# TencentYoutuResearch/ImageMatching-OETR

Measured on AMD Instinct MI355X. Metric: image-pairs/sec @640x640 (OETR hot path: feature correlation + overlap regression, features resident in HBM), higher is better.
Workload: dtype f32 (3xf16-split operands, fp32 accumulate); 1 GPU; BASELINE configs[1]: batch=8 pairs/GPU, 640x640 -> 20x20 tokens/image, C=256, 8 enc + 2 dec layers, f32_split_f16; pairs_per_gpu=8, global_pairs=8, streams=3, world_size=1, gpu_max_hw_queues=4, encoder_tile_rows=64, tail_mode=direct form (throughput setting for overlapped streams), parallelism=pairs sharded over 1 rank(s); all-gather of boxes only

## Files before the change

### imagematching_oetr_amd/csrc/api.hip

```cpp
#include <math.h>
#include <stdlib.h>
#include <string.h>

#include <string>
#include <vector>

#include "../../include/oetr_hip.h"
#include "common.h"

using namespace oetr;

constexpr int OETR_PREREDUCE_MIN_TOKENS = 768;
constexpr int OETR_DIRECT_TAIL_MIN_ROWS = 16000;

namespace {

thread_local std::string g_err;

oetr_status fail(oetr_status st, const std::string& msg) {
  g_err = msg;
  return st;
}
oetr_status hip_fail(hipError_t e, const char* what) {
  return fail(OETR_ERR_HIP, std::string(what) + ": " + hipGetErrorString(e));
// ... 94 lines not shown
struct oetr_trace {
  std::vector<hipEvent_t> ev;
  std::vector<int> kid;
  int used = 0;
  int dropped = 0;
};

struct oetr_ctx {
  oetr_trace* trace = nullptr;
  int device = 0;
  int mode = GM_SPLIT;
  int kv_prereduce = -1;
  mutable int dec_fault = 0;
  int dec_split = 0;
  int tail_mode = 0;
  int policy = 0;
  int enc_tile = 0;
  int attn_full = 0;
  int num_cus = 256;
  float* dev = nullptr;
  size_t dev_floats = 0;
  EncLayerDev enc[OETR_N_ENC];
  DecKVDev dkv;
  DecLayerDev dec[OETR_N_DEC];
  const float* qe[2];
  const float *dec_tgt1, *dec_q0, *dec_qkv1;
  HeadsDev heads;
};

struct oetr_neck_ctx {
  oetr_trace* trace = nullptr;
  int device = 0;
  int num_cus = 256;
  int conv_rows = 0;
  float* dev = nullptr;
  const f32x4 *proj_wh[2], *proj_wl[2];
  const float *proj_b, *ln_w, *ln_b;
  const f32x4 *conv_wh[3], *conv_wl[3];
  const f32x4 *conv_wh_rw[3], *conv_wl_rw[3];
  int conv_kernel = 0;
  const float* conv_b[3];
  const f32x4 *out_wh, *out_wl;
  const float* out_b;
};

namespace {

#ifdef OETR_PHASE_TIMING
long long* g_tbuf = nullptr;
#endif

struct Workspace {
  float *x, *qp, *pos, *kvp[2], *ksp[2], *att0, *z0, *dkv1, *dks1, *conv_out, *gn_part, *sm_part, *hs,
      *logits, *cxy, *tlbr, *convp, *kbuf[2], *vt[2], *kvr, *ksr;
  uint32_t* flags;
  size_t bytes;
};

bool make_geom(int n, int hf1, int wf1, int hf2, int wf2, Geom* g) {
  if (n <= 0 || hf1 <= 0 || wf1 <= 0 || hf2 <= 0 || wf2 <= 0) return false;
  const long L1 = (long)hf1 * wf1, L2 = (long)hf2 * wf2;
  if (L1 > OETR_MAX_TOKENS || L2 > OETR_MAX_TOKENS) return false;
  if ((long)n * (L1 + L2) > (1L << 30) / C) return false;
  g->N = n;
  g->L[0] = (int)L1; g->L[1] = (int)L2;
  g->hf[0] = hf1; g->wf[0] = wf1; g->hf[1] = hf2; g->wf[1] = wf2;
  g->nt[0] = (g->L[0] + TM - 1) / TM; g->nt[1] = (g->L[1] + TM - 1) / TM;
  g->row0[0] = 0; g->row0[1] = n * g->L[0];
  g->prow0[0] = 0; g->prow0[1] = g->L[0];
  g->tile0[0] = 0; g->tile0[1] = n * g->nt[0];
  g->ntiles = n * (g->nt[0] + g->nt[1]);
  g->rows = n * (g->L[0] + g->L[1]);
  return true;
}

int encoder_tile_rows(const oetr_ctx* h, const Geom& g) {
  if (!gm_half(h->mode) || h->attn_full) return TM;
  const int want = h->enc_tile;
  if (want == TM || want == 64) return want;
  return g.ntiles > h->num_cus ? 64 : TM;
}
Geom encoder_geom(const Geom& g, int rows) {
  Geom e = g;
  for (int i = 0; i < 2; ++i) e.nt[i] = (g.L[i] + rows - 1) / rows;
  e.tile0[0] = 0; e.tile0[1] = g.N * e.nt[0];
  e.ntiles = g.N * (e.nt[0] + e.nt[1]);
  return e;
}

Workspace carve(const Geom& g, void* base, bool attn_full = false) {
  Workspace w;
  size_t off = 0;
  auto take = [&](size_t floats) {
    float* p = base ? reinterpret_cast<float*>(static_cast<char*>(base) + off) : nullptr;
    off += (floats * sizeof(float) + 255) & ~size_t(255);
    return p;
  };
  const size_t rows = g.rows, nt = g.ntiles;
  w.flags = reinterpret_cast<uint32_t*>(take(OETR_WORKSPACE_STATUS_BYTES / sizeof(float)));
  w.x = take(rows * C);
  w.qp = take((rows + (size_t)2 * g.N * 64) * C);
  w.pos = take((size_t)(g.L[0] + g.L[1]) * C);
  for (int i = 0; i < 2; ++i) { w.kvp[i] = take(nt * KV_FLOATS); w.ksp[i] = take(nt * C); }
  w.att0 = take(nt * C); w.z0 = take(nt * NH);
  w.dkv1 = take(nt * KV_FLOATS); w.dks1 = take(nt * C);
  w.conv_out = take(rows * C);
  w.gn_part = take(nt * 32 * 2);
  w.sm_part = take(nt * 4);
  w.hs = take((size_t)2 * g.N * C);
  w.logits = take(rows);
  w.cxy = take((size_t)2 * g.N * 2);
  w.tlbr = take((size_t)2 * g.N * 4);
  w.convp = take((size_t)9 * rows * C);
  w.kvr = take((size_t)2 * g.N * KV_FLOATS);
  w.ksr = take((size_t)2 * g.N * C);
  for (int i = 0; i < 2; ++i) {
    w.kbuf[i] = attn_full ? take(rows * C) : nullptr;
    w.vt[i] = attn_full ? take((size_t)g.N * C * TM * (g.nt[0] + g.nt[1])) : nullptr;
  }
  w.bytes = off;
  return w;
}

oetr_status check_ws(const Geom& g, void* ws, size_t ws_bytes, Workspace* out, bool attn_full = false) {
  if (!ws) return fail(OETR_ERR_WORKSPACE, "workspace is NULL");
  if (reinterpret_cast<uintptr_t>(ws) & 255)
    return fail(OETR_ERR_WORKSPACE, "workspace must be 256-byte aligned");
  *out = carve(g, ws, attn_full);
  if (out->bytes > ws_bytes)
    return fail(OETR_ERR_WORKSPACE, "workspace too small: need " + std::to_string(out->bytes) +
                                        " bytes, got " + std::to_string(ws_bytes));
  return OETR_OK;
}

HeatLaunch heat_launch(const oetr_ctx* h, const Geom& g, const Workspace& w, const float* mem1,
                       const float* mem2, const float* hs1, const float* hs2, float* cxy1,
                       float* cxy2, int img_h1, int img_h2) {
  HeatLaunch p;
  p.g = g;
  p.w = h->heads;
  p.mem[0] = mem1; p.mem[1] = mem2;
  p.hs[0] = hs1; p.hs[1] = hs2;
  p.conv_out = w.conv_out;
  p.gn_part = w.gn_part;
  p.sm_part = w.sm_part;
  p.logits = w.logits;
  p.cxy[0] = cxy1; p.cxy[1] = cxy2;
  p.img_h[0] = img_h1; p.img_h[1] = img_h2;
  p.tlbr[0] = p.tlbr[1] = nullptr;
  p.box[0] = p.box[1] = nullptr;
  p.img_w[0] = p.img_w[1] = 0;
  p.flags = w.flags;
  p.publish = nullptr;
  p.force_staged_conv = h->tail_mode == 3;
  p.convp_units = 9;
  p.mask[0] = p.mask[1] = nullptr;
  return p;
}

oetr_status check_masks(const oetr_ctx* h, const float* mask1, const float* mask2, bool encoder) {
  if (!mask1 && !mask2) return OETR_OK;
  if (!mask1 || !mask2) return fail(OETR_ERR_BAD_ARG, "masks: pass both mask1 and mask2, or neither");
  if (encoder && ((h->mode != GM_SPLIT && h->mode != GM_F32) || h->attn_full))
    return fail(OETR_ERR_UNSUPPORTED, "masks: built for OETR_DTYPE_F32_SPLIT_F16, OETR_DTYPE_F32_SPLIT_QK16 and OETR_DTYPE_F32 with linear attention "
                                      "(the reference's FullAttention turns a masked query row into NaN, "
                                      "linear_attention.py:74-81)");
  return OETR_OK;
}
// ... 37 lines not shown
    }
  }
  if (h->dec_split == DEC_SPLIT_K && d.convp_units == 9 && beside_convp && gm_half(h->mode)) d.convp_units = 3;
  d.ksplit = (h->dec_split == DEC_SPLIT_K || (h->dec_split == 0 && fits)) && images <= DEC_SPLIT_MAX_IMAGES
                 ? DEC_SPLIT_K : 1;
  d.flags = w.flags;
  d.xch_epoch = w.flags + STATUS_EPOCH_WORD;
  d.xch = reinterpret_cast<unsigned long long*>(reinterpret_cast<char*>(w.flags) + STATUS_XCH_OFFSET);
  d.tbuf = nullptr;
  d.dbg = 0;
  if (d.ksplit == DEC_SPLIT_K && h->dec_fault) { d.dbg = DEC_DBG_FAULT; h->dec_fault = 0; }
#ifdef OETR_PHASE_TIMING
  d.tbuf = g_tbuf ? g_tbuf + 16 * 4096 : nullptr;
#endif
  return d;
}

oetr_status run_correlation(oetr_ctx* h, const Geom& g, const Workspace& w, const float* feat1,
                            const float* feat2, const float* pos1, const float* pos2,
                            int enc_layers, hipStream_t s, bool with_decoder = true,
                            bool resident = false, const float* mask1 = nullptr,
                            const float* mask2 = nullptr) {
  EncLaunch p;
  memset(&p, 0, sizeof(p));
  if (!resident) {
    p.feat_nchw[0] = feat1; p.feat_nchw[1] = feat2;
    p.pos_nchw[0] = pos1; p.pos_nchw[1] = pos2;
    p.pos_out = w.pos;
  }
  p.tile_rows = encoder_tile_rows(h, g);
  p.g = encoder_geom(g, p.tile_rows);
#ifdef OETR_ABLATE
  { const char* e = getenv("OETR_ABLATE"); p.dbg = e ? atoi(e) : 0; }
#endif
#ifdef OETR_PHASE_TIMING
  {
    static long long* tb = nullptr;
    if (!tb) (void)hipMalloc(&tb, sizeof(long long) * 16 * 65536);
    p.tbuf = tb;
    g_tbuf = tb;
  }
#endif
  p.x = w.x; p.qp = w.qp; p.pos = w.pos;
  p.mask[0] = mask1; p.mask[1] = mask2;
  p.flags = w.flags;
  p.attn_full = h->attn_full;
  p.policy = h->policy;
  for (int i = 0; i < 2; ++i) p.lpad[i] = g.nt[i] * TM;
  p.vt_off[0] = 0; p.vt_off[1] = (size_t)g.N * C * p.lpad[0];
  p.kbuf_out = w.kbuf[0]; p.vt_out = w.vt[0];
  p.a = h->enc[0];
  p.kv_out = w.kvp[0]; p.ks_out = w.ksp[0];
  int prereduce = h->attn_full ? 0 : h->kv_prereduce;
  if (prereduce < 0) prereduce = (g.L[0] >= OETR_PREREDUCE_MIN_TOKENS || g.L[1] >= OETR_PREREDUCE_MIN_TOKENS) ? 1 : 0;
  TRACED(h, s, K_ENC_A, launch_encoder(p, false, 0, h->mode, s));
  p.feat_nchw[0] = p.feat_nchw[1] = p.pos_nchw[0] = p.pos_nchw[1] = nullptr;
  for (int l = 0; l < enc_layers; ++l) {
    p.b = h->enc[l];
    p.b_cross = l & 1;
    p.kv_in = w.kvp[l & 1]; p.ks_in = w.ksp[l & 1];
    p.kv_reduced = 0;
    if (prereduce == 1) {
      TRACED(h, s, K_KV_REDUCE, launch_kv_reduce(p.g, w.kvp[l & 1], w.ksp[l & 1], w.kvr, w.ksr, s));
      p.kv_in = w.kvr; p.ks_in = w.ksr;
      p.kv_reduced = 1;
    }
    p.kbuf_in = w.kbuf[l & 1]; p.vt_in = w.vt[l & 1];
    int tail;
    if (l + 1 == OETR_N_ENC) {
      tail = 1;
      p.d = h->dkv;
      p.att0_out = w.att0; p.z0_out = w.z0; p.dkv1_out = w.dkv1; p.dks1_out = w.dks1;
      p.dec_q0 = h->dec_q0;
    } else if (l + 1 < enc_layers) {
      tail = 0;
      p.a = h->enc[l + 1];
      p.kv_out = w.kvp[(l + 1) & 1]; p.ks_out = w.ksp[(l + 1) & 1];
      p.kbuf_out = w.kbuf[(l + 1) & 1]; p.vt_out = w.vt[(l + 1) & 1];
    } else {
      tail = 2;
    }
    TRACED(h, s, tail == 0 ? K_ENC_BA : tail == 1 ? K_ENC_BDEC : K_ENC_B,
           launch_encoder(p, true, tail, h->mode, s));
  }
  if (enc_layers == OETR_N_ENC && with_decoder) {
    DecLaunch d = dec_launch(h, g, w);
    TRACED(h, s, K_DECODER, launch_decoder(d, s));
  }
  return OETR_OK;
}

oetr_status check_weight(const char* name, const float* w, size_t n, bool f16_range) {
  for (size_t i = 0; i < n; ++i) {
    const float a = fabsf(w[i]);
    if (!(a <= 3.4028234e38f))
      return fail(OETR_ERR_UNSUPPORTED, std::string(name) + ": non-finite weight at index " + std::to_string(i));
    if (f16_range && a >= 65504.0f)
      return fail(OETR_ERR_UNSUPPORTED, std::string(name) + ": |w| = " + std::to_string(a) +
                  " at index " + std::to_string(i) + " exceeds the f16 range of this dtype; use "
                  "OETR_DTYPE_BF16 or OETR_DTYPE_F32");
  }
  return OETR_OK;
}
#define CHECK_W(name, ptr, n, f16r)                                      \
  do {                                                                   \
    oetr_status rc__ = check_weight(name, ptr, n, f16r);                 \
    if (rc__) return rc__;                                               \
  } while (0)

oetr_status copy_out(float* dst, const float* src, size_t floats, hipStream_t s) {
  if (!dst) return OETR_OK;
  HIP_TRY(hipMemcpyAsync(dst, src, floats * sizeof(float), hipMemcpyDeviceToDevice, s));
  return OETR_OK;
}

}

extern "C" {

const char* oetr_last_error(void) { return g_err.c_str(); }
int oetr_abi_version(void) { return OETR_ABI_VERSION; }

oetr_status oetr_create(const oetr_weights* w, oetr_dtype dtype, int device, oetr_handle* out) {
  if (!w || !out) return fail(OETR_ERR_BAD_ARG, "oetr_create: NULL argument");
  if (w->struct_size != sizeof(oetr_weights) || w->abi_version != OETR_ABI_VERSION)
    return fail(OETR_ERR_BAD_ARG, "oetr_create: oetr_weights size/ABI mismatch");
  static_assert(OETR_WORKSPACE_STATUS_BYTES == STATUS_BYTES && OETR_FLAG_EXCHANGE == FLAG_EXCHANGE, "status block");
  static_assert(OETR_DTYPE_F32 == GM_F32 && OETR_DTYPE_F32_SPLIT_F16 == GM_SPLIT &&
                    OETR_DTYPE_F16 == GM_F16 && OETR_DTYPE_BF16 == GM_BF16, "oetr_dtype == GM_*");
  if (dtype != OETR_DTYPE_F32 && dtype != OETR_DTYPE_F32_SPLIT_F16 && dtype != OETR_DTYPE_F16 &&
// ... 992 lines not shown
```

### imagematching_oetr_amd/csrc/common.h

```cpp
#pragma once
#include <hip/hip_runtime.h>
#include <stdint.h>

#include <type_traits>

namespace oetr {

constexpr int C = 256;
constexpr int NH = 8;
constexpr int HD = 32;
constexpr int FF = 512;
constexpr int TM = 32;
constexpr int LDA = C + 4;
constexpr int LDH = FF + 4;
constexpr int NTHREADS = 256;
constexpr int KV_FLOATS = NH * HD * HD;
constexpr float LN_EPS = 1e-5f;
constexpr float ATTN_EPS = 1e-6f;
constexpr int MAX_TOKENS = 10000;

#ifdef OETR_ABLATE
#define ABL(flags, bit) (((flags) & (bit)) != 0)
#else
#define ABL(flags, bit) false
#endif
#if defined(OETR_ABLATE)
#define PHASE_STAMP(p, idx) do { if (((p).dbg >> 16) == (idx) + 1) return; } while (0)
#elif defined(OETR_PHASE_TIMING) && OETR_PHASE_TIMING == 2
#define PHASE_STAMP(p, idx)                                                              \
  do {                                                                                   \
    if ((threadIdx.x & 63) == 0 && blockIdx.x < 16 && (p).tbuf)                          \
      (p).tbuf[(blockIdx.x * 8 + (threadIdx.x >> 6)) * 16 + (idx)] = __builtin_amdgcn_s_memtime(); \
  } while (0)
#elif defined(OETR_PHASE_TIMING) && OETR_PHASE_TIMING == 3
#define PHASE_STAMP(p, idx)                                                              \
  do {                                                                                   \
    if (threadIdx.x == 0 && (p).tbuf) (p).tbuf[blockIdx.x * 16 + (idx)] = __builtin_amdgcn_s_memrealtime(); \
  } while (0)
#elif defined(OETR_PHASE_TIMING)
#define PHASE_STAMP(p, idx)                                                              \
  do {                                                                                   \
    if (threadIdx.x == 0 && (p).tbuf) (p).tbuf[blockIdx.x * 16 + (idx)] = __builtin_amdgcn_s_memtime(); \
  } while (0)
#else
#define PHASE_STAMP(p, idx) do {} while (0)
#endif
#if defined(OETR_ABLATE) && defined(OETR_PHASE_TIMING)
#error "OETR_ABLATE and OETR_PHASE_TIMING are separate builds"
#endif
enum { ABL_KVREDUCE = 1, ABL_GELU = 2, ABL_ELU = 4, ABL_LN = 8, ABL_GEMM = 16, ABL_STORE = 32,
       ABL_XLOAD = 64, ABL_WLOAD = 128, ABL_ATTN = 256, ABL_KVSTATE = 512 };

typedef float f32x4 __attribute__((ext_vector_type(4)));
typedef float f32x16 __attribute__((ext_vector_type(16)));
typedef _Float16 f16x8 __attribute__((ext_vector_type(8)));
typedef _Float16 f16x4 __attribute__((ext_vector_type(4)));
typedef _Float16 f16x2 __attribute__((ext_vector_type(2)));
typedef __bf16 bf16x8 __attribute__((ext_vector_type(8)));
typedef __bf16 bf16x2 __attribute__((ext_vector_type(2)));

#ifndef OETR_WT
#define OETR_WT 7
#endif
template <bool WT>
__device__ __forceinline__ void store16(float* base_uniform, unsigned byte_off, const f32x4& v) {
  if constexpr (WT) {
    typedef uint32_t u32x4_ __attribute__((ext_vector_type(4)));
    const __amdgpu_buffer_rsrc_t rs = __builtin_amdgcn_make_buffer_rsrc(base_uniform, 0, 0x7fffffff, 0x00020000);
    __builtin_amdgcn_raw_buffer_store_b128(__builtin_bit_cast(u32x4_, v), rs, (int)byte_off, 0, 16 );
  } else {
    *reinterpret_cast<f32x4*>(reinterpret_cast<char*>(base_uniform) + byte_off) = v;
  }
}

enum { GM_F32 = 0, GM_SPLIT = 1, GM_F16 = 2, GM_BF16 = 3 };
constexpr bool gm_half(int m) { return m != GM_F32; }
constexpr int gm_planes(int m) { return m == GM_SPLIT ? 2 : 1; }

enum { SITE_FULL = 0, SITE_ACT_HI = 1, SITE_W_HI = 2, SITE_HI = 3 };
constexpr bool site_w_lo(int s) { return s == SITE_FULL || s == SITE_ACT_HI; }
constexpr bool site_act_lo(int s) { return s == SITE_FULL || s == SITE_W_HI; }
constexpr int site_mfmas(int s) { return s == SITE_FULL ? 3 : s == SITE_HI ? 1 : 2; }
#ifndef OETR_SITE_Q
#define OETR_SITE_Q SITE_FULL
#endif
#ifndef OETR_SITE_K
#define OETR_SITE_K SITE_FULL
#endif
#ifndef OETR_SITE_V
#define OETR_SITE_V SITE_FULL
#endif
#ifndef OETR_SITE_MERGE
#define OETR_SITE_MERGE SITE_FULL
#endif
#ifndef OETR_SITE_MLP1
#define OETR_SITE_MLP1 SITE_FULL
#endif
#ifndef OETR_SITE_MLP2
#define OETR_SITE_MLP2 SITE_FULL
#endif
#ifndef OETR_SITE_DEC_K
#define OETR_SITE_DEC_K SITE_FULL
#endif
#ifndef OETR_SITE_DEC_V
#define OETR_SITE_DEC_V SITE_FULL
#endif
template <int POL> struct SitePolicy;
template <> struct SitePolicy<0> {
  static constexpr int Q = OETR_SITE_Q, K = OETR_SITE_K, V = OETR_SITE_V, MERGE = OETR_SITE_MERGE,
                       MLP1 = OETR_SITE_MLP1, MLP2 = OETR_SITE_MLP2, DEC_K = OETR_SITE_DEC_K,
                       DEC_V = OETR_SITE_DEC_V;
};
template <> struct SitePolicy<1> {
  static constexpr int Q = SITE_HI, K = SITE_HI, V = SITE_FULL, MERGE = SITE_FULL, MLP1 = SITE_FULL,
                       MLP2 = SITE_FULL, DEC_K = SITE_HI, DEC_V = SITE_FULL;
};
constexpr int N_POLICIES = 2;

constexpr float SPLIT_SCALE = 2048.0f;
constexpr float SPLIT_INV = 1.0f / 2048.0f;
constexpr int LDAH = C + 8;
constexpr int LDHH = FF + 8;

struct Geom {
  int N;
  int L[2];
// ... 135 lines not shown
#ifndef OETR_GEMM_U
#define OETR_GEMM_U 4
#endif
template <int K, int NT, int U = OETR_GEMM_U>
__device__ __forceinline__ void gemm_rows32(const float* __restrict__ A, int lda,
                                            const f32x4* __restrict__ Wp, int nt0,
                                            int lane, f32x16 (&acc)[NT], int dbg = 0) {
  if (ABL(dbg, ABL_GEMM)) return;
  constexpr int KS = K / 8;
  constexpr int NCH = KS / U;
  static_assert(KS % (2 * U) == 0, "K must be a multiple of 16*U");
  const float* a_ptr = A + (lane & 31) * lda + 4 * (lane >> 5);
  const f32x4* w_ptr[NT];
#pragma unroll
  for (int t = 0; t < NT; ++t) w_ptr[t] = Wp + (size_t)(nt0 + t) * KS * 64;

  constexpr int NB = 4, CPB = NCH / NB;
  static_assert(NCH % (2 * NB) == 0, "K must be a multiple of 16*U*NB");
  GemmRegs<NT, U> r0, r1;
  gemm_fetch<NT, U>(r0, a_ptr, w_ptr, 0, (unsigned)lane);
  for (int b = 0; b < NB; ++b) {
    f32x16 part[NT];
#pragma unroll
    for (int t = 0; t < NT; ++t) part[t] = f32x16{0};
    for (int c = b * CPB; c < (b + 1) * CPB; c += 2) {
      gemm_fetch<NT, U>(r1, a_ptr, w_ptr, c + 1, (unsigned)lane);
      __builtin_amdgcn_sched_barrier(0);
      gemm_mma<NT, U>(r0, part);
      __builtin_amdgcn_sched_barrier(0);
      if (c + 2 < NCH) gemm_fetch<NT, U>(r0, a_ptr, w_ptr, c + 2, (unsigned)lane);
      __builtin_amdgcn_sched_barrier(0);
      gemm_mma<NT, U>(r1, part);
      __builtin_amdgcn_sched_barrier(0);
    }
#pragma unroll
    for (int t = 0; t < NT; ++t) acc[t] += part[t];
  }
}

__device__ __forceinline__ void split2(float a, float b, f16x2& hi, f16x2& lo) {
  typedef float v2f __attribute__((ext_vector_type(2)));
  const v2f ab = v2f{a, b};
  hi = __builtin_convertvector(ab, f16x2);
  const v2f sc = ab * v2f{SPLIT_SCALE, SPLIT_SCALE};
  lo = __builtin_bit_cast(f16x2, __builtin_amdgcn_cvt_pkrtz(
                                     __builtin_fmaf((float)hi[0], -SPLIT_SCALE, sc[0]),
                                     __builtin_fmaf((float)hi[1], -SPLIT_SCALE, sc[1])));
}
constexpr uint32_t FLAG_F16_RANGE = 1u;
constexpr uint32_t FLAG_EXCHANGE = 2u;
constexpr uint32_t FLAG_PUBLISHED = 0x80000000u;
constexpr int DEC_SPLIT_K = 4, DEC_SPLIT_MAX_IMAGES = 16, DEC_SPLIT_EXCHANGES = 5;
constexpr int DEC_DBG_FAULT = 0x5a;
constexpr size_t STATUS_EPOCH_WORD = 16, STATUS_XCH_OFFSET = 256,
                 STATUS_XCH_BYTES = (size_t)DEC_SPLIT_MAX_IMAGES * DEC_SPLIT_EXCHANGES * DEC_SPLIT_K * 256 * 8,
                 STATUS_BYTES = STATUS_XCH_OFFSET + STATUS_XCH_BYTES;
constexpr float F16_MAX = 65504.0f;
constexpr bool gm_f16_range(int m) { return m == GM_SPLIT || m == GM_F16; }
typedef unsigned short u16x2 __attribute__((ext_vector_type(2)));
struct Range {
  uint32_t mx = 0;
  float fm = 0.f;
  __device__ __forceinline__ void see2(float a, float b) {
    fm = __builtin_fmaxf(__builtin_fmaxf(fm, __builtin_fabsf(a)), __builtin_fabsf(b));
  }
  __device__ __forceinline__ void see_hi(uint32_t hi_pair) {
    mx = __builtin_bit_cast(uint32_t, __builtin_elementwise_max(__builtin_bit_cast(u16x2, mx),
                                                                __builtin_bit_cast(u16x2, hi_pair & 0x7fff7fffu)));
  }
  __device__ __forceinline__ bool bad() const {
    return (mx & 0xffffu) >= 0x7c00u || (mx >> 16) >= 0x7c00u || !(fm < 65520.0f);
  }
};
template <int M>
__device__ __forceinline__ void range_report(const Range& rg, uint32_t* flags) {
  if constexpr (gm_f16_range(M)) {
    if (__builtin_amdgcn_ballot_w64(rg.bad()) != 0 && (threadIdx.x & 63) == 0) atomicOr(flags, FLAG_F16_RANGE);
  }
}
template <int M>
__device__ __forceinline__ void cvt_planes2(float a, float b, uint32_t& hi, uint32_t& lo, Range& rg) {
  if constexpr (M == GM_SPLIT) {
    f16x2 h, l;
    split2(a, b, h, l);
    hi = __builtin_bit_cast(uint32_t, h);
    lo = __builtin_bit_cast(uint32_t, l);
  } else if constexpr (M == GM_F16) {
    hi = __builtin_bit_cast(uint32_t, __builtin_convertvector(f32x2{a, b}, f16x2));
    lo = 0;
  } else {
    hi = __builtin_bit_cast(uint32_t, __builtin_convertvector(f32x2{a, b}, bf16x2));
    lo = 0;
  }
  if constexpr (gm_f16_range(M)) rg.see2(a, b);
}
template <int M>
__device__ __forceinline__ f32x16 mma16(const f32x4& a, const f32x4& b, const f32x16& c) {
  if constexpr (M == GM_BF16)
    return __builtin_amdgcn_mfma_f32_32x32x16_bf16(__builtin_bit_cast(bf16x8, a),
                                                   __builtin_bit_cast(bf16x8, b), c, 0, 0, 0);
  else
    return __builtin_amdgcn_mfma_f32_32x32x16_f16(__builtin_bit_cast(f16x8, a),
                                                  __builtin_bit_cast(f16x8, b), c, 0, 0, 0);
}
typedef uint32_t u32x4 __attribute__((ext_vector_type(4)));
__device__ __forceinline__ void split8(const f32x4& a0, const f32x4& a1, f32x4& hi, f32x4& lo,
// ... 523 lines not shown
                                               HAS_NEXT ? nW + noff : nullptr,
                                               HAS_NEXT ? nWl + noff : nullptr, a, acc, cross, epi);
    if constexpr (TWO && SITE != SITE_HI) {
#pragma unroll
      for (int mt = 0; mt < NMT; ++mt)
#pragma unroll
        for (int r = 0; r < 16; ++r) acc[mt][r] = fmaf(cross[mt][r], SPLIT_INV, acc[mt][r]);
    }
  }
};
typedef WStream2T<GM_SPLIT> WStream2;

#endif

int set_last_error(int status, const char* msg);
struct EncLayerDev {
  const f32x4 *wq, *wk, *wv, *wmerge, *w1, *w2;
  const f32x4 *wq_l, *wk_l, *wv_l, *wmerge_l, *w1_l, *w2_l;
  const float *lnq_w, *lnq_b, *lnkv_w, *lnkv_b, *ln2_w, *ln2_b;
};
struct DecKVDev {
  const f32x4 *wk[2], *wv[2];
  const f32x4 *wk_l[2], *wv_l[2];
  const float *bk[2], *bv[2];
};

struct EncLaunch {
  Geom g;
  float* x;
  float* qp;
  const float* pos;
  const float* kv_in;
  const float* ks_in;
  float* kv_out;
  float* ks_out;
  float* att0_out;
  float* z0_out;
  float* dkv1_out;
  float* dks1_out;
  const float* dec_q0;
  EncLayerDev b;
  EncLayerDev a;
  DecKVDev d;
  int attn_full;
  const float* kbuf_in;
  const float* vt_in;
  float* kbuf_out;
  float* vt_out;
  int lpad[2];
  size_t vt_off[2];
  int tile_rows;
  int b_cross;
  int kv_reduced;
  int policy;
  int dbg;
  long long* tbuf;
  uint32_t* flags;
  const float* feat_nchw[2];
  const float* pos_nchw[2];
  float* pos_out;
  const float* mask[2];
};

hipError_t launch_encoder(const EncLaunch& p, bool has_b, int tail, int mode, hipStream_t s);
hipError_t launch_kv_reduce(const Geom& g, const float* kvp, const float* ksp, float* kvr, float* ksr,
                            hipStream_t s);

struct MhaDev {
  const float *wq_t, *wk_t, *wv_t, *wm_t;
  const float *bq, *bk, *bv;
};
struct DecLayerDev {
  MhaDev self_attn, cross;
  const float *w1_t, *w2_t;
  const float *n1w, *n1b, *n2w, *n2b, *n3w, *n3b;
};
struct DecLaunch {
  Geom g;
  DecLayerDev layer[2];
  const float* qe[2];
  const float* tgt1;
  const float* qkv1;
  const float* att0_part;
  const float* z0_part;
  const float* dkv1;
  const float* dks1;
  float* hs;
  int convp_units;
  int ksplit;
  unsigned long long* xch;
  unsigned* xch_epoch;
  uint32_t* flags;
  long long* tbuf;
  int dbg;
};
struct DecConstLaunch {
  DecLayerDev layer[2];
  const float* qe[2];
  float *tgt1, *q0, *qkv1;
};
hipError_t launch_decoder_consts(const DecConstLaunch& p, hipStream_t s);
hipError_t launch_decoder(const DecLaunch& p, hipStream_t s);

struct HeadsDev {
  const f32x4* conv_w;
  const f32x4* conv_w_l;
// ... 97 lines not shown
```

### imagematching_oetr_amd/csrc/encoder.hip

```cpp
#include <type_traits>

#include "common.h"


#ifndef OETR_SOAK_AMP
#define OETR_SOAK_AMP 0
#endif
#ifndef OETR_SPLIT_STATE
#define OETR_SPLIT_STATE 1
#endif

namespace oetr {

constexpr int S0_OFF = 0;
constexpr int S1_OFF = S0_OFF + TM * LDA;
constexpr int H_OFF = S1_OFF + TILE_FLOATS;
constexpr int KSUM_OFF = H_OFF + HID_FLOATS;
constexpr int Z_OFF = KSUM_OFF + C;
constexpr int LNP_OFF = Z_OFF + TM * NH;
constexpr int SMEM_FLOATS = LNP_OFF + 6 * C;

template <int NW>
struct EncCfg {
  static constexpr int NT = 8 / NW;
// ... 739 lines not shown
        split8(v0, v1, bh, bl, rg);
        mma16_split3(ah, al, bh, bl, kv, c1);
        __builtin_amdgcn_sched_barrier(0);
      }
    };
    row_tile(std::integral_constant<int, 0>{});
    if constexpr (NMT == 2) {
      if (two) row_tile(std::integral_constant<int, 1>{});
    }
#if OETR_SOAK_AMP & 2
    __builtin_amdgcn_s_setprio(0);
#endif
#pragma unroll
    for (int r = 0; r < 16; ++r) kv[r] = fmaf(c1[r], SPLIT_INV, kv[r]);
  } else {
    auto row_tile = [&](auto MT_) {
      constexpr int mt = decltype(MT_)::value;
      auto operands = [&](int r, float& k, float& v) {
        float m;
        if constexpr (MASKED) m = msk_s[32 * mt + crow(r, half)];
        else m = 32 * mt + crow(r, 0) < nv2 ? 1.0f : 0.0f;
        const float x = accK[mt][r];
        k = (elu1(x)) * m;
        ksum += k;
        v = accV[mt][r] * (inv_len * m);
      };
      float kc, vc;
      operands(0, kc, vc);
#pragma unroll
      for (int r = 0; r < 16; ++r) {
        float kn = 0.f, vn = 0.f;
        if (r + 1 < 16) operands(r + 1, kn, vn);
        kv = __builtin_amdgcn_mfma_f32_32x32x2f32(kc, vc, kv, 0, 0, 0);
        __builtin_amdgcn_sched_barrier(0);
        kc = kn; vc = vn;
      }
    };
    row_tile(std::integral_constant<int, 0>{});
    if constexpr (NMT == 2) {
      if (two) row_tile(std::integral_constant<int, 1>{});
    }
  }
  ksum += __shfl_xor(ksum, 32, 64);
}
__device__ __forceinline__ void kv_state_write(const f32x16& kv, float ksum, int lane, int wave,
                                               float* __restrict__ kv_out,
                                               float* __restrict__ ks_out, int slot) {
  f32x4* dst = reinterpret_cast<f32x4*>(kv_out) + ((size_t)slot * NH + wave) * 4 * 64;
#pragma unroll
  for (int q = 0; q < 4; ++q) {
    f32x4 o = {kv[4 * q], kv[4 * q + 1], kv[4 * q + 2], kv[4 * q + 3]};
    store16<(OETR_WT & 4) != 0>(reinterpret_cast<float*>(dst), (q * 64 + (unsigned)lane) * 16u, o);
  }
  if (lane < 32) (ks_out + (size_t)slot * C + wave * HD)[(unsigned)lane] = ksum;
}

template <bool HAS_B, int TAIL, int MODE, int POL, int ROWS, int RTW = RT, bool MASKED = false>
__device__ __forceinline__ void encoder64_body(const EncLaunch& p, float* smem) {
  constexpr int NMT = RTW / 32, THREADS = 512, TPR = THREADS / RTW, F4 = 64 / TPR;
  using L2 = E2<RTW>;
  using SP = SitePolicy<POL>;
  float* R1f = smem + L2::R1;
  float* R2f = smem + L2::R2;
  Range rg;
  const PlanesT<MODE, RTW> P1(R1f, &rg), P2(R2f, &rg);
  float* Xf = HAS_B ? R2f : R1f;
  float* ksum_s = smem + L2::KSUM;
  float* lnp_s = smem + L2::LNP;
  float* lnx_s = smem + L2::LNX;
  using WS = WStream2T<MODE, ROWS, NMT>;
  WS ws;
  constexpr int P_MERGE = 0;
  constexpr int P_1A = WS::adv(P_MERGE), P_1B = WS::adv(P_1A), P_2A = WS::adv(P_1B), P_2B = WS::adv(P_2A);
  constexpr int P_T0 = HAS_B ? WS::adv(P_2B) : 0;
  constexpr int P_T1 = WS::adv(P_T0), P_T2 = WS::adv(P_T1), P_T3 = WS::adv(P_T2);

  const Geom& g = p.g;
  const int tid = threadIdx.x, lane = tid & 63, wave = __builtin_amdgcn_readfirstlane(tid >> 6);
  const int half = lane >> 5, col = lane & 31;
  const int wcol = 32 * wave;
  const int lrow = tid / TPR, lpart = tid % TPR;

  const int logical = xcd_remap(blockIdx.x, g.ntiles);
  const int per = g.nt[0] + g.nt[1];
  const int n = logical / per;
  const int rem = logical - n * per;
  const int side = rem >= g.nt[0];
  const int t_idx = side ? rem - g.nt[0] : rem;
  const int L = g.L[side];
  const int l0 = t_idx * RTW;
  const int nvalid = min(RTW, L - l0);
  const size_t row_base = (size_t)g.row0[side] + (size_t)n * L + l0;
  const int slot = g.tile0[side] + n * g.nt[side] + t_idx;
  const size_t qrow_base = (size_t)slot * RTW;
  const bool nchw = !HAS_B && p.feat_nchw[0] != nullptr;
  ws.set_rows(nvalid);
  ws.set_lane(lane);

  stage_ln_params<THREADS, HAS_B, TAIL>(lnp_s, p, tid);
  const f32x4* pos = reinterpret_cast<const f32x4*>(
                         p.pos + (size_t)(g.prow0[side] + l0 + min(lrow, nvalid - 1)) * C) + lpart;

  f32x16 xacc[NMT];
  PHASE_STAMP(p, 0);
  if (!HAS_B) PHASE_STAMP(p, 13);

  if (HAS_B) {
// ... 256 lines not shown
        P1.template put4<site_act_lo(SP::Q)>(lrow, 4 * (i * TPR + lpart), (xn[i] * qw[i * TPR] + qb[i * TPR]) + ps[i]);
        P2.template put4<site_act_lo(SP::K) || site_act_lo(SP::V)>(lrow, 4 * (i * TPR + lpart),
                                                                   (xn[i] * kw[i * TPR] + kb[i * TPR]) + ps[i]);
      }
    }
    __syncthreads();
    PHASE_STAMP(p, 9);
    f32x16 accQ[NMT] = {};
    ws.template gemm<C, P_T0, true, C, SP::Q, SP::K, true>(P1, p.a.wq, p.a.wq_l, wave, 0, lane, accQ, p.a.wk,
                                                           p.a.wk_l, wave, 0);
    PHASE_STAMP(p, 10);
    f32x16 accK[NMT] = {}, accV[NMT] = {};
    {
      f32x4* qf = reinterpret_cast<f32x4*>(p.qp + qrow_base * C) + (size_t)wave * NMT * 4 * 64;
      const bool two = ws.two();
      u32x4 qhi = {0, 0, 0, 0}, qlo = {0, 0, 0, 0};
      auto qepi = [&](auto CI_) {
        constexpr int CI = decltype(CI_)::value, mt = NMT == 2 ? CI / 8 : 0, pr = NMT == 2 ? CI % 8 : CI / 2;
        constexpr int s2 = pr / 4, j = pr % 4;
        if constexpr (NMT == 1 && CI % 2 == 1) return;
        if (mt == 1 && !two) return;
        const float qmask = MASKED ? lnx_s[32 * mt + col] : 1.0f;
        const float a = MASKED ? elu1(accQ[mt][2 * pr]) * qmask : elu1(accQ[mt][2 * pr]);
        const float b = MASKED ? elu1(accQ[mt][2 * pr + 1]) * qmask : elu1(accQ[mt][2 * pr + 1]);
        if constexpr (MODE == GM_BF16) {
          if constexpr (pr % 2 == 0) { qhi[0] = __builtin_bit_cast(uint32_t, a); qhi[1] = __builtin_bit_cast(uint32_t, b); }
          else {
            qhi[2] = __builtin_bit_cast(uint32_t, a); qhi[3] = __builtin_bit_cast(uint32_t, b);
            store16<(OETR_WT & 2) != 0>(reinterpret_cast<float*>(qf), ((mt * 4 + pr / 2) * 64 + (unsigned)lane) * 16u,
                                        __builtin_bit_cast(f32x4, qhi));
          }
        } else {
          uint32_t h, l;
          cvt_planes2<GM_SPLIT>(a, b, h, l, rg);
          qhi[j] = h; qlo[j] = l;
          if constexpr (j == 3) {
            store16<(OETR_WT & 2) != 0>(reinterpret_cast<float*>(qf), ((mt * 4 + 2 * s2) * 64 + (unsigned)lane) * 16u,
                                        __builtin_bit_cast(f32x4, qhi));
            store16<(OETR_WT & 2) != 0>(reinterpret_cast<float*>(qf), ((mt * 4 + 2 * s2 + 1) * 64 + (unsigned)lane) * 16u,
                                        __builtin_bit_cast(f32x4, qlo));
          }
        }
      };
      ws.template gemm_epi<C, P_T1, true, C, SP::K, SP::V>(P2, p.a.wk, p.a.wk_l, wave, 0, lane, accK, p.a.wv,
                                                           p.a.wv_l, wave, 0, qepi);
    }
    ws.template gemm<C, P_T2, false, C, SP::V>(P2, p.a.wv, p.a.wv_l, wave, 0, lane, accV, nullptr, nullptr,
                                               0, 0);
    PHASE_STAMP(p, 11);
    f32x16 kv;
    float ksum;
    kv_state_64<MODE, NMT, MASKED>(accK, accV, L, nvalid, half, ws.two(), kv, ksum, rg, lnx_s);
    kv_state_write(kv, ksum, lane, wave, p.kv_out, p.ks_out, slot);
    PHASE_STAMP(p, 12);
  } else if (TAIL == 1) {
    float bias_k[2], bias_v[2];
#pragma unroll
    for (int dl = 0; dl < 2; ++dl) {
      bias_k[dl] = p.d.bk[dl][wcol + col];
      bias_v[dl] = p.d.bv[dl][wcol + col];
    }
    {
      f32x4 xv[F4], ps[F4];
      const f32x4* src = reinterpret_cast<const f32x4*>(Xf + lrow * LDA) + lpart;
#pragma unroll
      for (int i = 0; i < F4; ++i) { xv[i] = src[i * TPR]; ps[i] = pos[i * TPR]; }
      __syncthreads();
#pragma unroll
      for (int i = 0; i < F4; ++i) {
        P1.template put4<site_act_lo(SP::DEC_K)>(lrow, 4 * (i * TPR + lpart), xv[i] + ps[i]);
        P2.template put4<site_act_lo(SP::DEC_V)>(lrow, 4 * (i * TPR + lpart), xv[i]);
      }
    }
    __syncthreads();
    auto dec_layer = [&](auto DL) {
      constexpr int dl = decltype(DL)::value;
      constexpr int PK = dl == 0 ? P_T0 : P_T2, PV = dl == 0 ? P_T1 : P_T3;
      f32x16 accK[NMT], accV[NMT];
#pragma unroll
      for (int mt = 0; mt < NMT; ++mt)
#pragma unroll
        for (int r = 0; r < 16; ++r) { accK[mt][r] = bias_k[dl]; accV[mt][r] = bias_v[dl]; }
      ws.template gemm<C, PK, true, C, SP::DEC_K, SP::DEC_V>(P1, p.d.wk[dl], p.d.wk_l[dl], wave, 0, lane, accK,
                                                             p.d.wv[dl], p.d.wv_l[dl], wave, 0);
      ws.template gemm<C, PV, false, C, SP::DEC_V>(P2, p.d.wv[dl], p.d.wv_l[dl], wave, 0, lane, accV, nullptr,
                                                   nullptr, 0, 0);
      f32x16 kv;
      float ksum;
      kv_state_64<MODE, NMT, MASKED>(accK, accV, L, nvalid, half, ws.two(), kv, ksum, rg, lnx_s);
      if constexpr (dl == 1) {
        kv_state_write(kv, ksum, lane, wave, p.dkv1_out, p.dks1_out, slot);
      } else {
        const float* q0 = p.dec_q0 + side * C + wave * HD;
        float a = 0.f;
#pragma unroll
        for (int r = 0; r < 16; ++r) a += q0[crow(r, half)] * kv[r];
        a += __shfl_xor(a, 32, 64);
        float z = q0[col] * ksum;
        z += __shfl_xor(z, 1, 64);
        z += __shfl_xor(z, 2, 64);
        z += __shfl_xor(z, 4, 64);
        z += __shfl_xor(z, 8, 64);
        z += __shfl_xor(z, 16, 64);
        if (half == 0) p.att0_out[(size_t)slot * C + wave * HD + col] = a;
        if (lane == 0) p.z0_out[(size_t)slot * NH + wave] = z;
        ws.template prime<C, P_T2, SP::DEC_K>(p.d.wk[1], p.d.wk_l[1], wave, 0, lane);
// ... 224 lines not shown
```

Baseline: 33080 image-pairs/s.

## Fuse KV-state prereduction into encoder via last-block atomic counter

Adds a third prereduce mode, used for the split-f16 path with 64-row tiles and small images. Each encoder block writes its partial KV state, then bumps a per-image atomic counter. The last block to finish sums all tile partials, read with sc1 buffer loads, into a ping-ponged reduced buffer. The next layer then reads a single reduced state per image instead of summing every tile's partial. This costs an extra serialized reduction inside one block per image and atomic and fence overhead, and it relies on write-through stores so the partials are visible to that block.

New measurement: 33240 image-pairs/s (median of 6 runs). About the same (+0.5%).

```diff
diff --git a/imagematching_oetr_amd/csrc/api.hip b/imagematching_oetr_amd/csrc/api.hip
--- a/imagematching_oetr_amd/csrc/api.hip
+++ b/imagematching_oetr_amd/csrc/api.hip
@@ -170,7 +170,7 @@
 
 struct Workspace {
   float *x, *qp, *pos, *kvp[2], *ksp[2], *att0, *z0, *dkv1, *dks1, *conv_out, *gn_part, *sm_part, *hs,
-      *logits, *cxy, *tlbr, *convp, *kbuf[2], *vt[2], *kvr, *ksr;
+      *logits, *cxy, *tlbr, *convp, *kbuf[2], *vt[2], *kvr[2], *ksr[2];
   uint32_t* flags;
   size_t bytes;
 };
@@ -230,8 +230,10 @@
   w.cxy = take((size_t)2 * g.N * 2);
   w.tlbr = take((size_t)2 * g.N * 4);
   w.convp = take((size_t)9 * rows * C);
-  w.kvr = take((size_t)2 * g.N * KV_FLOATS);
-  w.ksr = take((size_t)2 * g.N * C);
+  for (int i = 0; i < 2; ++i) {
+    w.kvr[i] = take((size_t)2 * g.N * KV_FLOATS);
+    w.ksr[i] = take((size_t)2 * g.N * C);
+  }
   for (int i = 0; i < 2; ++i) {
     w.kbuf[i] = attn_full ? take(rows * C) : nullptr;
     w.vt[i] = attn_full ? take((size_t)g.N * C * TM * (g.nt[0] + g.nt[1])) : nullptr;
@@ -375,7 +377,14 @@
   p.a = h->enc[0];
   p.kv_out = w.kvp[0]; p.ks_out = w.ksp[0];
   int prereduce = h->attn_full ? 0 : h->kv_prereduce;
-  if (prereduce < 0) prereduce = (g.L[0] >= OETR_PREREDUCE_MIN_TOKENS || g.L[1] >= OETR_PREREDUCE_MIN_TOKENS) ? 1 : 0;
+  if (prereduce < 0) {
+    if (g.L[0] >= OETR_PREREDUCE_MIN_TOKENS || g.L[1] >= OETR_PREREDUCE_MIN_TOKENS) prereduce = 1;
+    else prereduce = h->mode == GM_SPLIT && p.tile_rows == 64 && (size_t)2 * g.N <= STATUS_KV_CTR_MAX ? 2 : 0;
+  }
+  if (prereduce == 2) {
+    p.kv_ctr = w.flags + STATUS_KV_CTR_WORD;
+    p.kvr_out = w.kvr[0]; p.ksr_out = w.ksr[0];
+  }
   TRACED(h, s, K_ENC_A, launch_encoder(p, false, 0, h->mode, s));
   p.feat_nchw[0] = p.feat_nchw[1] = p.pos_nchw[0] = p.pos_nchw[1] = nullptr;
   for (int l = 0; l < enc_layers; ++l) {
@@ -384,8 +393,11 @@
     p.kv_in = w.kvp[l & 1]; p.ks_in = w.ksp[l & 1];
     p.kv_reduced = 0;
     if (prereduce == 1) {
-      TRACED(h, s, K_KV_REDUCE, launch_kv_reduce(p.g, w.kvp[l & 1], w.ksp[l & 1], w.kvr, w.ksr, s));
-      p.kv_in = w.kvr; p.ks_in = w.ksr;
+      TRACED(h, s, K_KV_REDUCE, launch_kv_reduce(p.g, w.kvp[l & 1], w.ksp[l & 1], w.kvr[0], w.ksr[0], s));
+      p.kv_in = w.kvr[0]; p.ks_in = w.ksr[0];
+      p.kv_reduced = 1;
+    } else if (prereduce == 2) {
+      p.kv_in = w.kvr[l & 1]; p.ks_in = w.ksr[l & 1];
       p.kv_reduced = 1;
     }
     p.kbuf_in = w.kbuf[l & 1]; p.vt_in = w.vt[l & 1];
@@ -399,6 +411,7 @@
       tail = 0;
       p.a = h->enc[l + 1];
       p.kv_out = w.kvp[(l + 1) & 1]; p.ks_out = w.ksp[(l + 1) & 1];
+      p.kvr_out = w.kvr[(l + 1) & 1]; p.ksr_out = w.ksr[(l + 1) & 1];
       p.kbuf_out = w.kbuf[(l + 1) & 1]; p.vt_out = w.vt[(l + 1) & 1];
     } else {
       tail = 2;
diff --git a/imagematching_oetr_amd/csrc/common.h b/imagematching_oetr_amd/csrc/common.h
--- a/imagematching_oetr_amd/csrc/common.h
+++ b/imagematching_oetr_amd/csrc/common.h
@@ -72,6 +72,25 @@
     *reinterpret_cast<f32x4*>(reinterpret_cast<char*>(base_uniform) + byte_off) = v;
   }
 }
+template <bool WT>
+__device__ __forceinline__ void store4(float* base_uniform, unsigned byte_off, float v) {
+  if constexpr (WT) {
+    const __amdgpu_buffer_rsrc_t rs = __builtin_amdgcn_make_buffer_rsrc(base_uniform, 0, 0x7fffffff, 0x00020000);
+    __builtin_amdgcn_raw_buffer_store_b32(__builtin_bit_cast(uint32_t, v), rs, (int)byte_off, 0, 16 );
+  } else {
+    *reinterpret_cast<float*>(reinterpret_cast<char*>(base_uniform) + byte_off) = v;
+  }
+}
+__device__ __forceinline__ f32x4 load16_sc1(const float* base_uniform, unsigned byte_off) {
+  const __amdgpu_buffer_rsrc_t rs =
+      __builtin_amdgcn_make_buffer_rsrc(const_cast<float*>(base_uniform), 0, 0x7fffffff, 0x00020000);
+  return __builtin_bit_cast(f32x4, __builtin_amdgcn_raw_buffer_load_b128(rs, (int)byte_off, 0, 16 ));
+}
+__device__ __forceinline__ float load4_sc1(const float* base_uniform, unsigned byte_off) {
+  const __amdgpu_buffer_rsrc_t rs =
+      __builtin_amdgcn_make_buffer_rsrc(const_cast<float*>(base_uniform), 0, 0x7fffffff, 0x00020000);
+  return __builtin_bit_cast(float, __builtin_amdgcn_raw_buffer_load_b32(rs, (int)byte_off, 0, 16 ));
+}
 
 enum { GM_F32 = 0, GM_SPLIT = 1, GM_F16 = 2, GM_BF16 = 3 };
 constexpr bool gm_half(int m) { return m != GM_F32; }
@@ -313,6 +332,7 @@
 constexpr uint32_t FLAG_PUBLISHED = 0x80000000u;
 constexpr int DEC_SPLIT_K = 4, DEC_SPLIT_MAX_IMAGES = 16, DEC_SPLIT_EXCHANGES = 5;
 constexpr int DEC_DBG_FAULT = 0x5a;
+constexpr size_t STATUS_KV_CTR_WORD = 32, STATUS_KV_CTR_MAX = 32;
 constexpr size_t STATUS_EPOCH_WORD = 16, STATUS_XCH_OFFSET = 256,
                  STATUS_XCH_BYTES = (size_t)DEC_SPLIT_MAX_IMAGES * DEC_SPLIT_EXCHANGES * DEC_SPLIT_K * 256 * 8,
                  STATUS_BYTES = STATUS_XCH_OFFSET + STATUS_XCH_BYTES;
@@ -942,6 +962,9 @@
   int tile_rows;
   int b_cross;
   int kv_reduced;
+  uint32_t* kv_ctr;
+  float* kvr_out;
+  float* ksr_out;
   int policy;
   int dbg;
   long long* tbuf;
diff --git a/imagematching_oetr_amd/csrc/encoder.hip b/imagematching_oetr_amd/csrc/encoder.hip
--- a/imagematching_oetr_amd/csrc/encoder.hip
+++ b/imagematching_oetr_amd/csrc/encoder.hip
@@ -815,7 +815,55 @@
     f32x4 o = {kv[4 * q], kv[4 * q + 1], kv[4 * q + 2], kv[4 * q + 3]};
     store16<(OETR_WT & 4) != 0>(reinterpret_cast<float*>(dst), (q * 64 + (unsigned)lane) * 16u, o);
   }
-  if (lane < 32) (ks_out + (size_t)slot * C + wave * HD)[(unsigned)lane] = ksum;
+  if (lane < 32) store4<(OETR_WT & 4) != 0>(ks_out + (size_t)slot * C + wave * HD, 4u * (unsigned)lane, ksum);
+}
+
+static_assert((OETR_WT & 4) != 0, "the in-launch state reduction reads partials stored sc1");
+__device__ __forceinline__ void kv_reduce_last(const EncLaunch& p, int side, int n, int tid, int lane, int wave,
+                                               float* flag_s) {
+  const Geom& g = p.g;
+  asm volatile("s_waitcnt vmcnt(0)" ::: "memory");
+  __syncthreads();
+  if (tid == 0) {
+    const uint32_t old = __hip_atomic_fetch_add(p.kv_ctr + side * g.N + n, 1u, __ATOMIC_RELAXED,
+                                                __HIP_MEMORY_SCOPE_AGENT);
+    const bool last = old + 1 == (uint32_t)g.nt[side];
+    if (last) __hip_atomic_store(p.kv_ctr + side * g.N + n, 0u, __ATOMIC_RELAXED, __HIP_MEMORY_SCOPE_AGENT);
+    flag_s[0] = last ? 1.f : 0.f;
+  }
+  __syncthreads();
+  if (!__builtin_amdgcn_readfirstlane(flag_s[0] != 0.f ? 1 : 0)) return;
+  const int nts = g.nt[side], slot0 = g.tile0[side] + n * nts, img = side * g.N + n;
+  const float* kvp = p.kv_out + ((size_t)slot0 * NH + wave) * (KV_FLOATS / NH);
+  const float* ksp = p.ks_out + (size_t)slot0 * C + wave * HD;
+  constexpr int KVR = 7;
+  constexpr unsigned TILE_KV = KV_FLOATS * 4, TILE_KS = C * 4;
+  f32x4 acc[4];
+#pragma unroll
+  for (int e = 0; e < 4; ++e) acc[e] = f32x4{0.f, 0.f, 0.f, 0.f};
+  float ks = 0.f;
+  for (int ti0 = 0; ti0 < nts; ti0 += KVR) {
+    f32x4 tmp[KVR][4];
+    float kt[KVR];
+#pragma unroll
+    for (int u = 0; u < KVR; ++u) {
+      const unsigned ti = (unsigned)min(ti0 + u, nts - 1);
+#pragma unroll
+      for (int e = 0; e < 4; ++e) tmp[u][e] = load16_sc1(kvp, ti * TILE_KV + (unsigned)(e * 64 + lane) * 16u);
+      kt[u] = load4_sc1(ksp, ti * TILE_KS + 4u * (unsigned)(lane & 31));
+    }
+#pragma unroll
+    for (int u = 0; u < KVR; ++u)
+      if (ti0 + u < nts) {
+#pragma unroll
+        for (int e = 0; e < 4; ++e) acc[e] += tmp[u][e];
+        ks += kt[u];
+      }
+  }
+  float* kvr = p.kvr_out + ((size_t)img * NH + wave) * (KV_FLOATS / NH);
+#pragma unroll
+  for (int e = 0; e < 4; ++e) store16<true>(kvr, (unsigned)(e * 64 + lane) * 16u, acc[e]);
+  if (lane < 32) store4<true>(p.ksr_out + (size_t)img * C + wave * HD, 4u * (unsigned)lane, ks);
 }
 
 template <bool HAS_B, int TAIL, int MODE, int POL, int ROWS, int RTW = RT, bool MASKED = false>
@@ -1178,6 +1226,7 @@
     float ksum;
     kv_state_64<MODE, NMT, MASKED>(accK, accV, L, nvalid, half, ws.two(), kv, ksum, rg, lnx_s);
     kv_state_write(kv, ksum, lane, wave, p.kv_out, p.ks_out, slot);
+    if (p.kv_ctr) kv_reduce_last(p, side, n, tid, lane, wave, ksum_s);
     PHASE_STAMP(p, 12);
   } else if (TAIL == 1) {
     float bias_k[2], bias_v[2];
```
